# ChenWu98/cycle-diffusion

Measured on AMD Instinct MI355X. Metric: images/sec, SD-v1.4 512px CycleDiffusion 100+100 steps, 1/2/4/8 MI355X, higher is better.
Workload: dtype fp16

## Files before the change

cycle-diffusion_amd/csrc/capi_ops.hip:

```cpp
#include "capi_internal.h"

namespace {

bf16_t* op_rows16(cd_engine* h, const float* src, int64_t rows, int C) {
  bf16_t* d = (bf16_t*)h->arena.alloc((size_t)rows * C * 2);
  launch_nchw_to_nhwc(h->st, src, d, (int)rows, C, 1, C, 1.f, 0.f, 0);
  return d;
}
Act op_image16(Ctx& c, const float* x, int B, int C, int H, int W, int Cpad) {
  Act a = alloc_act(c, B, H, W, Cpad);
  launch_nchw_to_nhwc(c.st, x, a.p, B, C, H * W, Cpad, 1.f, 0.f, 0);
  return a;
}

bf16_t* op_nan_rows16(cd_engine* h, int64_t rows, int ld) {
  const size_t bytes = (size_t)(rows + 64) * ld * 2;
  bf16_t* t = (bf16_t*)h->arena.alloc(bytes);
  HIP_CHECK(hipMemsetAsync(t, 0xFF, bytes, h->st));
  return t;
}
float* op_nan_buffer(cd_engine* h, size_t n) {
  float* t = (float*)h->arena.alloc(n * sizeof(float));
  launch_fill_f32(h->st, t, __builtin_nanf(""), (int64_t)n);
  return t;
// ... 11 lines not shown

Act op_rows_view(const void* p, int B, int T, int C, int ld, bool f32) {
  Act a; a.p = (bf16_t*)const_cast<void*>(p); a.B = B; a.H = T; a.W = 1; a.C = C; a.ld = ld; a.f32 = f32;
  return a;
}
Act op_upload_rows(cd_engine* h, const float* x, int64_t rows, int C, int pad) {
  const int ld = C + pad;
  float* t = op_nan_buffer(h, (size_t)rows * ld);
  op_put_cols(h, t, ld, 0, x, rows, C);
  return op_rows_view(t, (int)rows, 1, C, ld, true);
}

const float* op_nchw_guarded(cd_engine* h, const float* x, int B, int C, int Czero, int ld, int HW) {
  if (ld == C) return x;
  float* t = op_nan_buffer(h, (size_t)B * ld * HW);
  if (Czero > C)
    HIP_CHECK(hipMemset2DAsync(t + (size_t)C * HW, (size_t)ld * HW * 4, 0, (size_t)(Czero - C) * HW * 4, B, h->st));
  HIP_CHECK(hipMemcpy2DAsync(t, (size_t)ld * HW * 4, x, (size_t)C * HW * 4, (size_t)C * HW * 4, B, hipMemcpyDeviceToDevice,
                             h->st));
  return t;
}
Act op_upload_nhwc(cd_engine* h, const float* x, int B, int C, int Czero, int ld, int H, int W) {
  const int HW = H * W;
  Act a; a.B = B; a.H = H; a.W = W; a.C = Czero; a.ld = ld; a.f32 = true;
  a.p = (bf16_t*)h->arena.alloc((size_t)B * HW * ld * sizeof(float));
  launch_nchw_to_nhwc_f32(h->st, op_nchw_guarded(h, x, B, C, Czero, ld, HW), a.pf(), B, ld, HW, ld, 1.f, 0.f);
  return a;
}
Act op_upload_nhwc16(cd_engine* h, const float* x, int B, int C, int ld, int H, int W, int Czero = 0) {
  const int HW = H * W;
  if (Czero < C) Czero = C;
  Act a; a.B = B; a.H = H; a.W = W; a.C = C; a.ld = ld;
  a.p = (bf16_t*)h->arena.alloc((size_t)B * HW * ld * sizeof(bf16_t));
  launch_nchw_to_nhwc(h->st, op_nchw_guarded(h, x, B, C, Czero, ld, HW), a.p, B, ld, HW, ld, 1.f, 0.f, 0);
  return a;
}
Act op_upload_nhwc_split(cd_engine* h, const float* x, int B, int C, int Cpad, int H, int W) {
  Act a; a.B = B; a.H = H; a.W = W; a.C = Cpad; a.ld = 2 * Cpad; a.f32 = true; a.split = true;
  a.p = (bf16_t*)h->arena.alloc((size_t)B * H * W * 2 * Cpad * sizeof(bf16_t));
  launch_nchw_to_nhwc_f32(h->st, x, a.pf(), B, C, H * W, Cpad, 1.f, 0.f, 1, h->overflow_dev);
  return a;
}

void op_download_nchw(cd_engine* h, const void* p, bool f32, int ld, float* y, int B, int C, int HW) {
  launch_nhwc_to_nchw(h->st, p, f32 ? 1 : 0, ld, y, B, C, HW, 1.f, 0.f);
}
void op_download(cd_engine* h, const Act& o, size_t floats, void* y) {
  HIP_CHECK(hipMemcpyAsync(y, o.p, floats * 4, hipMemcpyDeviceToDevice, h->st));
  HIP_CHECK(hipStreamSynchronize(h->st));
  h->check_overflow();
}

void conv_out_hw(int H, int W, int KH, int KW, int stride, int pad, bool asym, bool up, int* Ho, int* Wo) {
  const int Hin = up ? 2 * H : H, Win = up ? 2 * W : W;
  *Ho = asym ? (Hin + 1 - KH) / stride + 1 : (Hin + 2 * pad - KH) / stride + 1;
  *Wo = asym ? (Win + 1 - KW) / stride + 1 : (Win + 2 * pad - KW) / stride + 1;
}
Ctx prec_ctx(cd_engine* h, int precision) {
  Ctx c = h->ctx();
  c.f32 = precision != 0; c.x3 = precision == 2;
  return c;
}

void op_conv2d(cd_handle h, const float* x0, int C0, const float* x1, int C1, int B, int H, int W,
               const void* packed_w, int N, int KH, int KW, int stride, int pad, int asym_pad, int up,
               const float* bias, const float* rowvec, const float* resid, int act, int tile, bool out16,
               float* y, float* stats) {
  CD_CHECK(h && x0 && packed_w && y, "bad argument");
  ArenaScope arena_scope(h->arena);
  Ctx c = h->ctx();
  if (up && out16) {
    ConvW* pw = (ConvW*)const_cast<void*>(packed_w);
    h->op_params.add_up_phase(pw);
    h->op_params.refresh_up_phase(h->st, pw);
  }
  ConvW w = *(const ConvW*)packed_w;
  CD_CHECK(w.N == N && w.KH == KH && w.KW == KW, "packed weight does not match the call");
  w.b = const_cast<float*>(bias);
  Act a0 = op_image16(c, x0, B, C0, H, W, x1 ? C0 : round_up(C0, 32));
  Act a1;
  if (x1) a1 = op_image16(c, x1, B, C1, H, W, C1);
  ConvOpts o; o.stride = stride; o.pad = pad; o.asym = asym_pad != 0; o.up = up != 0; o.tile = tile;
  if (act & 0x400) {
    CD_CHECK(out16 && conv_ln_fold_available(c, w, (int64_t)B * H * W) , "LayerNorm fold needs tile 30 shapes");
    o.ln_fold = true;
    act &= ~0x400;
  }
  o.act = act;
  o.out_f32 = !out16;
  o.want_stats = stats != nullptr;
  int Ho, Wo;
  conv_out_hw(H, W, KH, KW, stride, pad, asym_pad != 0, up != 0, &Ho, &Wo);
  const int Nout = w.geglu ? N / 2 : N;
  if (rowvec) { o.rowvec = rowvec; o.rowvec_ld = N; o.rows_per_vec = Ho * Wo; }
  Act r;
  if (resid) {
    r = op_image16(c, resid, B, Nout, Ho, Wo, Nout);
    o.resid = &r;
  }
  Act out = conv_fwd(c, w, a0, x1 ? &a1 : nullptr, o);
  op_download_nchw(h, out.p, !out16, out.ld, y, B, Nout, Ho * Wo);
  if (stats) {
    CD_CHECK(out.stats, "this convolution produces no GroupNorm statistics (GEGLU, or rows %% 32 != 0)");
    HIP_CHECK(hipMemcpyAsync(stats, out.stats, (size_t)(out.rows() / 32) * 2 * Nout * sizeof(float),
                             hipMemcpyDeviceToDevice, h->st));
  }
}

void op_cross_attention_ctrl(cd_engine* h, const float* q_own, const float* q_src, const float* k_own,
                             const float* k_src, const float* v_own, const float* mapper, const float* alpha,
                             const float* weight, int B, int B_src, int B_ctrl, int H, int Tq, int L, int L_buf, int D,
                             float scale, int q_log2, int opad, float* o) {
  CD_CHECK(h && q_own && q_src && k_own && k_src && v_own && mapper && alpha && weight && o, "bad argument");
  CD_CHECK(B > 0 && B_src > 0 && B_ctrl > 0 && H > 0 && Tq > 0 && D > 0 && L > 0 && L_buf >= L, "bad argument");
  CD_CHECK(opad >= 0 && opad % 4 == 0, "opad: a multiple of 4 elements");
  ArenaScope arena_scope(h->arena);
  const int C = H * D, ldo = C + opad;
  CtrlAttnParams p;
  p.q_own = op_rows16(h, q_own, (int64_t)B * Tq, C); p.q_src = op_rows16(h, q_src, (int64_t)B_src * Tq, C);
  p.k_own = op_rows16(h, k_own, (int64_t)B * L_buf, C); p.k_src = op_rows16(h, k_src, (int64_t)B_src * L_buf, C);
  const bf16_t* vb16 = op_rows16(h, v_own, (int64_t)B * L, C);
  bf16_t* va = (bf16_t*)h->arena.alloc((size_t)B * L * C * 2);
  bf16_t* vb = (bf16_t*)h->arena.alloc((size_t)B * L * C * 2);
  launch_ctrl_values(h->st, vb16, mapper, alpha, weight, B, B_ctrl, L, C, va, vb);
  bf16_t* ob = op_nan_rows16(h, (int64_t)B * Tq, ldo);
  p.va = va; p.vb = vb; p.o = ob;
  p.B = B; p.B_src = B_src; p.H = H; p.Tq = Tq; p.L = L; p.D = D;
  p.ldq = C; p.ldk = C; p.ldv = C; p.ldo = ldo;
  p.q_bs = (int64_t)Tq * C; p.k_bs = (int64_t)L_buf * C; p.v_bs = (int64_t)L * C; p.o_bs = (int64_t)Tq * ldo;
  p.scale = scale; p.q_log2 = q_log2 != 0;
  launch_cross_attention_ctrl(h->st, p);
  op_download_nchw(h, ob, false, ldo, o, B * Tq, ldo, 1);
}

}

extern "C" {

int cd_op_pack_conv_weight(cd_handle h, const float* w_host, int N, int Cin, int KH, int KW, int geglu,
                           void** packed_dev, int* Npad, int* Cpad) {
  CD_API_BEGIN
  enter_engine(h);
  CD_CHECK(h && w_host && packed_dev, "bad argument");
  static int counter = 0;
  ConvW* c = h->op_params.new_conv(N, Cin, KH, KW, false, geglu != 0);
  const std::string name = "op." + std::to_string(counter++);
  h->op_params.conv_weight(name, c);
  int64_t shape[4] = {N, Cin, KH, KW};
  h->op_params.load(h->st, name, w_host, 4, shape);
  *packed_dev = c;
  if (Npad) *Npad = c->Npad;
  if (Cpad) *Cpad = c->Cpad;
  CD_API_END
}

int cd_op_free(cd_handle, void*) { return 0; }

int cd_op_conv2d(cd_handle h, const float* x0, int C0, const float* x1, int C1, int B, int H, int W,
                 const void* packed_w, int N, int KH, int KW, int stride, int pad, int asym_pad, int up,
                 const float* bias, const float* rowvec, const float* resid, int act, int tile, float* y) {
  CD_API_BEGIN
  enter_engine(h);
  op_conv2d(h, x0, C0, x1, C1, B, H, W, packed_w, N, KH, KW, stride, pad, asym_pad, up, bias, rowvec, resid, act, tile,
            false, y, nullptr);
  CD_API_END
}

// ... 973 lines not shown
```

cycle-diffusion_amd/csrc/engine.h:

```cpp
#pragma once
#include <map>
#include <memory>
#include <string>
#include <vector>

#include "common.h"
#include "kernels.h"
#include "../../include/cyclediff.h"

namespace cd {

class Arena {
 public:
  ~Arena();
  void init(size_t bytes);
  void* alloc(size_t bytes);
  size_t mark() const { return off_; }
  void release(size_t m) { off_ = m; }
  void reset() { off_ = 0; }
  size_t capacity() const { return cap_; }
  size_t high_water() const { return high_; }
 private:
  char* base_ = nullptr;
  size_t cap_ = 0, off_ = 0, high_ = 0;
// ... 48 lines not shown
  ~ParamStore();
  bool f32 = false;
  bool x3 = false;
  int* overflow = nullptr;
  int version = 0;
  ConvW* new_conv(int N, int Cin, int KH, int KW, bool bias, bool geglu = false);
  float* new_vec(int n, float init = 0.f);
  void add_up_phase(ConvW* c);
  void refresh_up_phase(hipStream_t st, ConvW* c);
  ParamDecl& declare(const std::string& name, std::vector<int64_t> shape);
  void conv_weight(const std::string& name, ConvW* c, int ref_ndim = 0, float scale = 1.f);
  void conv_weight_t(const std::string& name, ConvW* c);
  void conv_bias(const std::string& name, ConvW* c);
  void conv_rows(const std::string& name, std::vector<int64_t> shape, ConvW* c, int dst_row0, int rows,
                 int src_base, int grp, int grp_stride, float scale = 1.f);
  void bias_rows(const std::string& name, int64_t n_total, float* dst, int dst_off, int rows, int src_base,
                 int grp, int grp_stride);
  void vec(const std::string& name, float* dst, int n);
  void mat_f32(const std::string& name, float* dst, int N, int K, int dst_row0 = 0);

  void load(hipStream_t st, const std::string& name, const float* host, int ndim, const int64_t* shape);
  int missing(std::string* first = nullptr) const;
  const std::vector<std::unique_ptr<ParamDecl>>& decls() const { return decls_; }
  size_t device_bytes() const { return dev_bytes_; }
 private:
  std::vector<std::unique_ptr<ParamDecl>> decls_;
  std::map<std::string, ParamDecl*> by_name_;
  std::vector<std::unique_ptr<ConvW>> convs_;
  std::vector<void*> allocs_;
  float* staging_ = nullptr;
  size_t staging_bytes_ = 0;
  size_t dev_bytes_ = 0;
  void* dmalloc(size_t bytes);
};

struct Ctx {
  hipStream_t st = nullptr;
  Arena* arena = nullptr;
  const bf16_t* zeros = nullptr;
  float* gn_partial = nullptr;
  size_t gn_partial_floats = 0;
  bool f32 = false;
  bool x3 = false;
  int* overflow = nullptr;
};
class PrecisionScope {
 public:
  PrecisionScope(Ctx& c, bool f32, bool x3) : c_(c), f32_(c.f32), x3_(c.x3) { c.f32 = f32; c.x3 = x3; }
  ~PrecisionScope() { c_.f32 = f32_; c_.x3 = x3_; }
  PrecisionScope(const PrecisionScope&) = delete;
  PrecisionScope& operator=(const PrecisionScope&) = delete;
 private:
  Ctx& c_;
  const bool f32_, x3_;
};

struct ConvOpts {
  int stride = 1;
  int pad = 1;
  bool asym = false;
  bool up = false;
  const float* rowvec = nullptr; int rowvec_ld = 0; int rows_per_vec = 1;
  const Act* resid = nullptr;
  int act = ACT_NONE;
  float alpha = 1.f;
  bool out_f32 = false;
  void* out = nullptr;
  int out_ld = 0;
  bool ln_fold = false;
  float ln_eps = 1e-5f;
  bool raw_geglu = false;
  bool want_stats = false;
  float* out_stats = nullptr;
  int tile = 0;
};
Act attention_flash_f32_fwd(Ctx& c, const float* q, int ldq, const float* k, int ldk, int64_t k_bs, const float* v, int ldv,
                            int64_t v_bs, int B, int H, int Tq, int Tk, int D, float scale, int Himg, int Wimg, bool q_log2);
Act geglu_f32_fwd(Ctx& c, const Act& h);
Act split_rows_f32_fwd(Ctx& c, const Act& x, const Act* x2 = nullptr);
Act alloc_act(Ctx& c, int B, int H, int W, int C, bool with_stats = false);
Act conv_fwd(Ctx& c, const ConvW& w, const Act& x, const Act* x2, const ConvOpts& o);
bool conv_up_phase_taken(const Ctx& c, const ConvW& w, const Act& x, const Act* x2, const ConvOpts& o);
bool conv_ln_fold_available(const Ctx& c, const ConvW& w, int64_t rows);

struct GNW { float* g = nullptr; float* b = nullptr; int C = 0; float eps = 1e-5f; };
Act groupnorm_fwd(Ctx& c, const GNW& w, const Act& x, const Act* x2, bool silu, const float* film = nullptr,
                  int film_ld = 0);
struct LNW { float* g = nullptr; float* b = nullptr; int C = 0; };
Act layernorm_fwd(Ctx& c, const LNW& w, const Act& x);
const float* groupnorm_coef_fwd(Ctx& c, const GNW& w, const Act& x);
GNW make_gn(ParamStore& ps, const std::string& pfx, int C, float eps);
LNW make_ln(ParamStore& ps, const std::string& pfx, int C);
ConvW* make_conv(ParamStore& ps, const std::string& pfx, int N, int Cin, int k, bool bias = true, bool geglu = false,
                 int ref_ndim = 4, float wscale = 1.f);
Act net_input_act(const void* p, int B, int H, int W, int C, bool f32, bool x3);

struct ResW {
  int cin = 0, cout = 0;
  bool up = false, down = false, film = false;
  GNW gn1, gn2;
  ConvW *conv1 = nullptr, *conv2 = nullptr, *skip = nullptr;
  int emb_off = -1;
};
Act res_fwd(Ctx& c, const ResW& r, const Act& x, const Act* x2, const float* proj, int proj_ld, bool t_shared);

struct AttnW {
  int C = 0, heads = 1;
  GNW norm;
  ConvW *qk = nullptr, *v = nullptr, *proj = nullptr;
  float* vbias = nullptr;
};
Act attn_block_fwd(Ctx& c, const AttnW& a, const Act& x);

enum {
  ST_ENTRY_QKV = 1,
  ST_ENTRY_LN1 = 2,
  ST_ENTRY_GN = 4,
};
int st_entry_stages();
bool st_entry_available(const Ctx& c, int64_t rows, int hw);
constexpr int64_t kStEntryNetMinRows = 61440;
struct StEntryW {
  GNW norm; LNW ln1;
  const ConvW *proj_in = nullptr, *qk1 = nullptr, *v1 = nullptr;
  ConvW *qkv = nullptr, *qkv_ln = nullptr;
  const float* vbias = nullptr;
};
void st_entry_alloc(ParamStore& ps, StEntryW& w);
void st_entry_refresh(hipStream_t st, StEntryW& w);
struct StEntryOut { Act h, qk; bf16_t* vt = nullptr; int Tpad = 0; int stages = 0; };
void vt_gemm_fwd(Ctx& c, const ConvW& wv, const bf16_t* x, int ldx, int B, int T, int Tpad, bf16_t* vt);
struct AtCoreOut { Act o; bf16_t* vt = nullptr; int Tpad = 0; int branch = 0; };
AtCoreOut at_core(Ctx& c, const ConvW& wv, const float* vbias, const Act& qk, const Act& n, int C, int heads, Act o = Act());
Act st_entry_proj_in(Ctx& c, const StEntryW& w, const Act& x, int stages);
StEntryOut st_entry_qkv(Ctx& c, const StEntryW& w, const Act& h, int stages);
StEntryOut st_entry_fwd(Ctx& c, const StEntryW& w, const Act& x, int stages);

Act avgpool2_fwd(Ctx& c, const Act& x);
Act upsample2_fwd(Ctx& c, const Act& x);
Act attention_f32_fwd(Ctx& c, const Act& qk, const Act& v, int H, int D, float scale, const float* obias);

Act attention_fwd(Ctx& c, const bf16_t* q, int ldq, const bf16_t* k, int ldk, const bf16_t* v, int ldv, int B,
                  int H, int Tq, int Tk, int D, float scale, int Himg, int Wimg, bool q_log2 = false, int rows = -1);
Act attention_vt_fwd(Ctx& c, const bf16_t* q, int ldq, const bf16_t* k, int ldk, const bf16_t* vt, int B,
                     int H, int Tq, int Tk, int Tpad, int D, float scale, int Himg, int Wimg, bool q_log2 = false,
                     const float* obias = nullptr, Act o = Act());

class Net {
 public:
  virtual ~Net() {}
  ParamStore params;
  cd_net_desc desc;
  bool f32 = false;
  bool x3 = false;
  void set_precision(const cd_net_desc& d) {
    f32 = d.precision == CD_PREC_F32 || d.precision == CD_PREC_F32X3;
    x3 = d.precision == CD_PREC_F32X3;
    params.f32 = f32; params.x3 = x3;
  }
  virtual int kind() const = 0;
};

struct TimeEmb {
  int mode = 0, dim = 0, hidden = 0;
  float *w0 = nullptr, *b0 = nullptr, *w1 = nullptr, *b1 = nullptr;
  float* proj_w = nullptr; float* proj_b = nullptr;
// ... 91 lines not shown
```

cycle-diffusion_amd/csrc/engine.hip:

```cpp
#include <limits.h>
#include <stdlib.h>

#include "engine.h"

#include <string.h>

namespace cd {

Arena::~Arena() { if (base_) (void)hipFree(base_); }
void Arena::init(size_t bytes) {
  if (base_) { (void)hipFree(base_); base_ = nullptr; }
  HIP_CHECK(hipMalloc((void**)&base_, bytes));
  cap_ = bytes; off_ = 0; high_ = 0;
}
void* Arena::alloc(size_t bytes) {
  size_t a = (off_ + 255) & ~(size_t)255;
  CD_CHECK(a + bytes <= cap_, "workspace arena exhausted: need %zu more bytes (capacity %zu); "
           "create the engine with a larger workspace", a + bytes - cap_, cap_);
  off_ = a + bytes;
  if (off_ > high_) high_ = off_;
  return base_ + a;
}

ParamStore::~ParamStore() {
// ... 272 lines not shown
  p.wgt = w.wphase; p.Ktot = 4 * w.Cpad; p.N = w.N;
  p.alpha = o.alpha; p.bias = w.b;
  p.rowvec = o.rowvec; p.rowvec_ld = o.rowvec_ld; p.rows_per_vec = o.rows_per_vec;
  Act y; y.B = x.B; y.H = 2 * x.H; y.W = 2 * x.W; y.C = w.N; y.f32 = false;
  if (o.out) { y.p = (bf16_t*)o.out; y.ld = o.out_ld; }
  else { y.ld = w.N; y.p = (bf16_t*)c.arena->alloc((size_t)p.M * w.N * 2); }
  if (o.out && o.out_stats) y.stats_buf = o.out_stats;
  else if (!o.out && o.want_stats) y.stats_buf = (float*)c.arena->alloc((size_t)(p.M / 32) * 2 * w.N * sizeof(float));
  p.stats = y.stats_buf;
  y.stats = y.stats_buf;
  const size_t mk = c.arena->mark();
  bf16_t* tmp = (bf16_t*)c.arena->alloc((size_t)p.M * w.N * 2);
  p.out = tmp; p.out_ld = w.N;
  p.zeros = c.zeros; p.tile = o.tile;
  launch_conv_gemm(c.st, p);
  launch_up_phase_reorder(c.st, tmp, y.p, x.B, x.H, x.W, w.N, y.ld);
  c.arena->release(mk);
  return y;
}

Act conv_fwd(Ctx& c, const ConvW& w, const Act& x, const Act* x2, const ConvOpts& o) {
  if (conv_up_phase_taken(c, w, x, x2, o)) return conv_up_phase_fwd(c, w, x, o);
  if (x.split) {
    CD_CHECK(!x2, "conv: a split activation cannot be concatenated");
    return conv_split_fwd(c, w, x, o);
  }
  ConvGemmParams p;
  CD_CHECK(w.f32 == c.f32 && x.f32 == c.f32 && (!x2 || x2->f32 == c.f32) && (!o.resid || o.resid->f32 == c.f32),
           "conv: operand precision does not match the running network");
  CD_CHECK((!x2 || !x2->split) && (!o.resid || !o.resid->split), "conv: split activation as a second source / residual");
  p.src0 = x.p; p.C0 = round_up(x.C, 32); p.ld0 = x.ld;
  if (x2) {
    CD_CHECK(x2->B == x.B && x2->H == x.H && x2->W == x.W, "conv: concat sources differ in shape");
    p.src1 = x2->p; p.C1 = x2->C; p.ld1 = x2->ld;
    CD_CHECK(x.C % 32 == 0 && x2->C % 32 == 0, "conv: concat channels must be multiples of 32");
  }
  CD_CHECK(p.C0 + p.C1 == w.Cpad, "conv: input channels %d+%d do not match weight Cpad %d", p.C0, p.C1, w.Cpad);
  CD_CHECK(x.ld >= p.C0, "conv: source row shorter than padded channel count");
  p.B = x.B; p.Hs = x.H; p.Ws = x.W; p.up = o.up ? 1 : 0;
  p.Hin = o.up ? x.H * 2 : x.H; p.Win = o.up ? x.W * 2 : x.W;
  p.KH = w.KH; p.KW = w.KW; p.stride = o.stride;
  if (o.asym) { p.pad_t = 0; p.pad_l = 0; p.Hout = (p.Hin + 1 - w.KH) / o.stride + 1; p.Wout = (p.Win + 1 - w.KW) / o.stride + 1; }
  else {
    p.pad_t = o.pad; p.pad_l = o.pad;
    p.Hout = (p.Hin + 2 * o.pad - w.KH) / o.stride + 1;
    p.Wout = (p.Win + 2 * o.pad - w.KW) / o.stride + 1;
  }
  p.M = x.B * p.Hout * p.Wout;
  p.wgt = w.w; p.wgt_frag = w.wfrag; p.Ktot = w.Ktot(); p.N = w.N;
  p.alpha = o.alpha; p.bias = w.b;
  p.rowvec = o.rowvec; p.rowvec_ld = o.rowvec_ld; p.rows_per_vec = o.rows_per_vec;
  const bool fuse_geglu = w.geglu && !o.raw_geglu;
  p.act = fuse_geglu ? ACT_GEGLU : o.act;
  const int Nout = fuse_geglu ? w.N / 2 : w.N;
  Act y; y.B = x.B; y.H = p.Hout; y.W = p.Wout; y.C = Nout; y.f32 = c.f32;
  if (o.out) { y.p = (bf16_t*)o.out; y.ld = o.out_ld; }
  else {
    y.ld = Nout;
    y.p = (bf16_t*)c.arena->alloc((size_t)p.M * Nout * ((o.out_f32 || c.f32) ? 4 : 2));
  }
  if (o.resid) {
    CD_CHECK(o.resid->rows() == p.M && o.resid->C == Nout, "conv: residual shape mismatch");
    p.resid = o.resid->p; p.resid_ld = o.resid->ld;
  }
  p.out = y.p; p.out_ld = y.ld; p.out_f32 = o.out_f32 ? 1 : 0;
  p.zeros = c.zeros; p.tile = o.tile;
  if (o.ln_fold) { p.ln_fold = 1; p.ln_eps = o.ln_eps; p.tile = kLinStreamTile; }
  if (c.f32) {
    p.out_f32 = 1;
    launch_conv_gemm_f32(c.st, p);
    return y;
  }
  if (!w.geglu && !o.out_f32 && ((p.Hout * p.Wout) % 32) == 0) {
    if (o.out && o.out_stats) y.stats_buf = o.out_stats;
    else if (!o.out && o.want_stats)
      y.stats_buf = (float*)c.arena->alloc((size_t)(p.M / 32) * 2 * Nout * sizeof(float));
    p.stats = y.stats_buf;
    y.stats = y.stats_buf;
  }
  launch_conv_gemm(c.st, p);
  return y;
}

bool conv_ln_fold_available(const Ctx& c, const ConvW& w, int64_t rows) {
  static const bool on = [] { const char* e = getenv("CYCLEDIFF_LN_FOLD"); return !(e && e[0] == '0'); }();
  static const int64_t min_rows = [] { const char* e = getenv("CYCLEDIFF_LN_FOLD_MIN_ROWS"); return e ? atoll(e) : 32768ll; }();
  return on && !c.f32 && w.wfrag && w.KH == 1 && w.KW == 1 && w.Cpad == 320 && rows >= min_rows && rows % 32 == 0 &&
         w.N % 64 == 0 && w.N <= 2560;
}

Act groupnorm_fwd(Ctx& c, const GNW& w, const Act& x, const Act* x2, bool silu, const float* film,
                  int film_ld) {
  GroupNormParams p;
  p.x = x.p; p.C0 = x.C; p.ld0 = x.ld;
  if (x2) { p.x1 = x2->p; p.C1 = x2->C; p.ld1 = x2->ld; }
  const int C = p.C0 + p.C1;
  CD_CHECK(C == w.C, "groupnorm: channels %d != weight %d", C, w.C);
  p.B = x.B; p.HW = x.H * x.W; p.G = 32; p.eps = w.eps; p.gamma = w.g; p.beta = w.b;
  p.film = film; p.film_ld = film_ld; p.silu = silu ? 1 : 0;
  Act y = alloc_act(c, x.B, x.H, x.W, C);
  p.y = y.p;
  if (c.f32) {
    CD_CHECK(x.f32 && (!x2 || x2->f32) && !x.split && (!x2 || !x2->split), "groupnorm: operand precision");
    if (c.x3) { p.split_out = 1; p.overflow = c.overflow; y.split = true; y.ld = 2 * C; }
    if (x.stats && x.ld == x.C && (!x2 || (x2->stats && x2->ld == x2->C))) {
      p.pre0 = x.stats;
      p.pre1 = x2 ? x2->stats : nullptr;
    }
    const size_t mk = c.arena->mark();
    void* ws = c.arena->alloc(groupnorm_f32_workspace(p.B, p.HW, C));
    launch_groupnorm_f32(c.st, p, ws);
    c.arena->release(mk);
    return y;
  }
  p.S = groupnorm_slabs(p.B, p.HW, C);
  const size_t part_floats = round_up((size_t)p.B * p.S * p.G * 2, (size_t)64);
  CD_CHECK(part_floats + (size_t)p.B * 2 * C <= c.gn_partial_floats, "groupnorm: workspace too small");
  p.partial = c.gn_partial;
  p.coef = c.gn_partial + part_floats;
  if (x.stats && x.ld == x.C && (!x2 || (x2->stats && x2->ld == x2->C))) {
    p.pre0 = x.stats;
    p.pre1 = x2 ? x2->stats : nullptr;
  }
  launch_groupnorm(c.st, p);
  return y;
}

const float* groupnorm_coef_fwd(Ctx& c, const GNW& w, const Act& x) {
  CD_CHECK(!c.f32 && !x.f32 && !x.split && x.C == w.C, "groupnorm coefficients: 16-bit single source of %d channels", w.C);
  GroupNormParams p;
  p.x = x.p; p.C0 = x.C; p.ld0 = x.ld;
  p.B = x.B; p.HW = x.H * x.W; p.G = 32; p.eps = w.eps; p.gamma = w.g; p.beta = w.b;
  p.no_apply = 1;
  p.S = groupnorm_slabs(p.B, p.HW, x.C);
  const size_t part_floats = round_up((size_t)p.B * p.S * p.G * 2, (size_t)64);
  CD_CHECK(part_floats + (size_t)p.B * 2 * x.C <= c.gn_partial_floats, "groupnorm: workspace too small");
  p.partial = c.gn_partial;
  p.coef = c.gn_partial + part_floats;
  if (x.stats && x.ld == x.C) p.pre0 = x.stats;
  launch_groupnorm(c.st, p);
  return p.coef;
}

int st_entry_stages() {
  static const int v = [] {
    const char* e = getenv("CYCLEDIFF_ST_ENTRY");
    int s = e && e[0] ? atoi(e) : (ST_ENTRY_QKV | ST_ENTRY_LN1 | ST_ENTRY_GN);
    if (!(s & ST_ENTRY_QKV)) s &= ~ST_ENTRY_LN1;
    return s;
  }();
  return v;
}

bool st_entry_available(const Ctx& c, int64_t rows, int hw) {
  return !c.f32 && rows >= 32768 && lin_stream_entry_supports(rows, hw, 320);
}

void st_entry_alloc(ParamStore& ps, StEntryW& w) {
  if (!w.qk1 || !w.v1 || !w.qk1->wfrag || !w.v1->wfrag || w.qk1->Cpad != 320 || w.qk1->N != 640 || w.v1->N != 320) return;
  w.qkv = ps.new_conv(960, 320, 1, 1, true);
  w.qkv_ln = ps.new_conv(960, 320, 1, 1, true);
}

void st_entry_refresh(hipStream_t st, StEntryW& w) {
  if (!w.qkv) return;
  const size_t row = (size_t)320 * sizeof(bf16_t);
  HIP_CHECK(hipMemcpyAsync(w.qkv->w, w.qk1->w, 640 * row, hipMemcpyDeviceToDevice, st));
  HIP_CHECK(hipMemcpyAsync(w.qkv->w + (size_t)640 * 320, w.v1->w, 320 * row, hipMemcpyDeviceToDevice, st));
  HIP_CHECK(hipMemsetAsync(w.qkv->b, 0, 960 * sizeof(float), st));
  if (w.vbias) HIP_CHECK(hipMemcpyAsync(w.qkv->b + 640, w.vbias, 320 * sizeof(float), hipMemcpyDeviceToDevice, st));
  launch_pack_wfrag(st, w.qkv->w, 320, w.qkv->wfrag, 960);
// ... 329 lines not shown
```

cycle-diffusion_amd/csrc/lin_stream.hip:

```cpp
#include <stdlib.h>

#include <mutex>

#include "common.h"
#include "kernels.h"

namespace cd {
namespace lin_detail {

typedef __attribute__((address_space(3))) void* lptr_t;
typedef __attribute__((ext_vector_type(4))) unsigned int u32x4;

constexpr int K = 320, NKS = K / 16, KSH = NKS / 2;
constexpr int WPIECE = 2 * KSH * 1024, WSLOTS = 3;
constexpr int APIECE = 128 * 128, ASLOTS = 3;
constexpr int NAP = 10;
constexpr int ST_LD = 36, ST_BYTES = 32 * ST_LD * 4;
constexpr int BIAS_MAX = 2560;
constexpr int OFF_A = WSLOTS * WPIECE, OFF_ST = OFF_A + ASLOTS * APIECE, OFF_BIAS = OFF_ST + 8 * ST_BYTES;
constexpr int LDS_BYTES = OFF_BIAS + BIAS_MAX * 4;
static_assert(LDS_BYTES <= 160 * 1024, "LDS");
constexpr unsigned kNoLoad = 0x80000000u;

__device__ __forceinline__ void wait_vmcnt_le(int n) {
// ... 19 lines not shown
}

__device__ __forceinline__ u32x4 load16_hidden(u32x4 rsrc, unsigned voff) {
  u32x4 r;
  asm volatile("buffer_load_dwordx4 %0, %1, %2, 0 offen" : "=v"(r) : "v"(voff), "s"(rsrc) : "memory");
  return r;
}
__device__ __forceinline__ uint4 pack8_sat(const float* f) {
#if CD_ACT_FP16
  typedef __attribute__((ext_vector_type(2))) _Float16 h2;
  uint32_t w[4];
#pragma unroll
  for (int i = 0; i < 4; ++i) {
    const h2 v = {(_Float16)__builtin_amdgcn_fmed3f(f[2 * i], -65504.0f, 65504.0f),
                  (_Float16)__builtin_amdgcn_fmed3f(f[2 * i + 1], -65504.0f, 65504.0f)};
    w[i] = __builtin_bit_cast(uint32_t, v);
  }
  return make_uint4(w[0], w[1], w[2], w[3]);
#else
  return pack8(f);
#endif
}
__device__ __forceinline__ void touch4(u32x4& a, u32x4& b, u32x4& c, u32x4& d) {
  asm volatile("" : "+v"(a), "+v"(b), "+v"(c), "+v"(d)::"memory");
}

template <int ACT, bool RESID, bool STATS, bool LNF = false, bool VT = false, bool GNA = false>
__global__ __launch_bounds__(512, 2) void k_lin_stream(LinStreamParams p) {
#if defined(__HIP_DEVICE_COMPILE__)
  constexpr bool GEGLU = (ACT == ACT_GEGLU);
  static_assert(!(GEGLU && (RESID || STATS)), "GEGLU has neither residual nor statistics");
  static_assert(!(VT && (GEGLU || RESID || STATS)) && !(GNA && (LNF || VT)), "entry variants are plain projections");
  extern __shared__ __attribute__((aligned(16))) char smem[];
  char* wring = smem;
  char* aring = smem + OFF_A;
  const int tid = threadIdx.x, lane = tid & 63;
  const int wave = __builtin_amdgcn_readfirstlane(tid >> 6);
  float* stage = (float*)(smem + OFF_ST + wave * ST_BYTES);
  float* bias_s = (float*)(smem + OFF_BIAS);
  const int mi = lane & 31, half = lane >> 5;
  const bool w_issuer = wave < 4;
  const int wq = wave & 3;

  const int NT = p.N >> 6;
  const int I = 2 * NT;
  const int nstrips = (p.M + 255) >> 8;
  const int G = gridDim.x;
  const int my_count = (nstrips - (int)blockIdx.x + G - 1) / G;
  if (my_count <= 0) return;
  const int cs = I >= 80 ? 4 : (I >= 40 ? 2 : 1);

  const __amdgpu_buffer_rsrc_t rs_a =
      __builtin_amdgcn_make_buffer_rsrc((void*)p.a, 0, (unsigned)((size_t)p.M * p.lda * 2), 0x00020000);
  const __amdgpu_buffer_rsrc_t rs_w =
      __builtin_amdgcn_make_buffer_rsrc((void*)p.wfrag, 0, (unsigned)((size_t)p.N * K * 2), 0x00020000);
  const __amdgpu_buffer_rsrc_t rs_o = __builtin_amdgcn_make_buffer_rsrc(
      (void*)p.out, 0, (unsigned)((size_t)p.M * p.ldo * 2), 0x00020000);
  const __amdgpu_buffer_rsrc_t rs_v = __builtin_amdgcn_make_buffer_rsrc(
      (void*)(VT ? p.vt : p.out), 0, VT ? (unsigned)p.vt_bytes : 0u, 0x00020000);
  u32x4 rs_r = {0u, 0u, 0u, 0x00020000u};
  if (RESID) {
    const uint64_t ra = (uint64_t)p.resid;
    rs_r[0] = (unsigned)ra; rs_r[1] = (unsigned)(ra >> 32) & 0xffffu;
    rs_r[2] = (unsigned)((size_t)p.M * p.ldr * 2);
  }

  for (int i = tid; i < p.N; i += 512) bias_s[i] = p.bias ? p.bias[i] : 0.f;

  auto issue_a = [&](int row0, int j, int slot) {
    const unsigned a_row = (unsigned)((lane >> 3) * p.lda * 2);
#pragma unroll
    for (int u = 0; u < 4; ++u) {
      const int x = wq * 4 + u;
      const unsigned a_lane = a_row + (unsigned)(((lane & 7) ^ ((4 * u + (lane >> 4)) & 7)) * 16);
      const unsigned base = (unsigned)(((row0 + 128 * (j & 1) + 8 * x) * p.lda + (j >> 1) * 64) * 2);
      __builtin_amdgcn_raw_ptr_buffer_load_lds(rs_a, (lptr_t)(aring + slot * APIECE + x * 1024), 16, a_lane + base, 0,
                                               0, 0);
    }
  };
  int w_boff[5];
#pragma unroll
  for (int u = 0; u < 5; ++u) {
    const int x = wq + 4 * u;
    w_boff[u] = ((x / KSH) * NKS + (x % KSH)) * 1024;
  }
  auto issue_w = [&](int piece, bool valid, int slot) {
    const int base = ((piece >> 1) * 2 * NKS + (piece & 1) * KSH) * 1024;
    const unsigned voff = valid ? (unsigned)(lane * 16) : kNoLoad;
#pragma unroll
    for (int u = 0; u < 5; ++u)
      __builtin_amdgcn_raw_ptr_buffer_load_lds(rs_w, (lptr_t)(wring + slot * WPIECE + (wq + 4 * u) * 1024), 16, voff,
                                               base + w_boff[u], 0, 0);
  };

  bf16x8 af[NKS], afn[NKS];
  auto normalise_rows = [&]() __attribute__((always_inline)) {
    float s1 = 0.f, s2 = 0.f;
#pragma unroll
    for (int ks = 0; ks < NKS; ++ks) {
      float f[8];
      unpack8(__builtin_bit_cast(uint4, af[ks]), f);
#pragma unroll
      for (int e = 0; e < 8; ++e) { s1 += f[e]; s2 = __builtin_fmaf(f[e], f[e], s2); }
      __builtin_amdgcn_sched_barrier(0);
    }
    s1 += __shfl_xor(s1, 32);
    s2 += __shfl_xor(s2, 32);
    const float mean = s1 * (1.0f / K);
    const float var = fmaxf(s2 * (1.0f / K) - mean * mean, 0.f);
    const float rstd = __builtin_amdgcn_rsqf(var + p.ln_eps);
    const float nmr = -mean * rstd;
#pragma unroll
    for (int ks = 0; ks < NKS; ++ks) {
      float f[8];
      unpack8(__builtin_bit_cast(uint4, af[ks]), f);
#pragma unroll
      for (int e = 0; e < 8; ++e) f[e] = __builtin_fmaf(f[e], rstd, nmr);
      af[ks] = __builtin_bit_cast(bf16x8, pack8_sat(f));
      __builtin_amdgcn_sched_barrier(0);
    }
  };
  auto gn_apply_rows = [&](int row0) __attribute__((always_inline)) {
    typedef __attribute__((ext_vector_type(8))) float f32x8s;
    const float* cf = p.gn_coef + (int64_t)(row0 / p.hw) * (2 * K);
    const bool hi = (lane >> 5) != 0;
#pragma unroll
    for (int ks = 0; ks < NKS; ++ks) {
      float f[8], cc[2][8];
#pragma unroll
      for (int ab = 0; ab < 2; ++ab) {
        f32x8s c0, c1;
        if (ab == 0)
          asm volatile("s_load_dwordx8 %0, %2, %3\n\ts_load_dwordx8 %1, %2, %4\n\ts_waitcnt lgkmcnt(0)"
                       : "=&s"(c0), "=&s"(c1) : "s"(cf), "n"(ks * 64), "n"(ks * 64 + 32) : "memory");
        else
          asm volatile("s_load_dwordx8 %0, %2, %3\n\ts_load_dwordx8 %1, %2, %4\n\ts_waitcnt lgkmcnt(0)"
                       : "=&s"(c0), "=&s"(c1) : "s"(cf), "n"(K * 4 + ks * 64), "n"(K * 4 + ks * 64 + 32) : "memory");
#pragma unroll
        for (int e = 0; e < 8; ++e) {
          cc[ab][e] = hi ? c1[e] : c0[e];
          asm volatile("" : "+v"(cc[ab][e]));
        }
      }
      unpack8(__builtin_bit_cast(uint4, af[ks]), f);
#pragma unroll
      for (int e = 0; e < 8; ++e) f[e] = f[e] * cc[0][e] + cc[1][e];
      af[ks] = __builtin_bit_cast(bf16x8, pack8(f));
      asm volatile("" : "+v"(af[ks]));
      __builtin_amdgcn_sched_barrier(0);
    }
  };
  auto take_a = [&](int j, int slot) {
    if ((j & 1) != (wave >> 2)) return;
    const int row = wq * 32 + mi;
    const int sw = (row >> 1) & 7;
    unsigned base = (unsigned)(OFF_A + slot * APIECE + row * 128 + ((half ^ sw) << 4));
    asm volatile("" : "+v"(base));
    const int kb = j >> 1;
#pragma unroll
    for (int c = 0; c < 5; ++c) {
      if (kb == c) {
#pragma unroll
        for (int f = 0; f < 4; ++f) afn[4 * c + f] = *(const bf16x8*)(smem + (base ^ (unsigned)(32 * f)));
        asm volatile("" ::: "memory");
      }
    }
  };

  int seq = 0;
  int wm0 = 0, wm1 = 0;
// ... 8 lines not shown
    if (is_o < my_count && is_gi <= gi) {
      if (!w_issuer) {
        issue_a(is_row0, is_j, is_slot);
        seq += 4;
        am0 = a_fly == 0 ? seq : am0;
        am1 = a_fly == 0 ? am1 : seq;
      }
      const bool wrap = is_j == NAP - 1;
      const int step_in = is_o == 0 ? 1 : cs, step_wrap = is_o == 0 ? I - 12 * cs + 3 : I - 9 * cs;
      ++a_fly;
      ++e_issue;
      is_slot = is_slot == ASLOTS - 1 ? 0 : is_slot + 1;
      is_gi += wrap ? step_wrap : step_in;
      is_j = wrap ? 0 : is_j + 1;
      is_o += wrap ? 1 : 0;
      is_row0 += wrap ? G * 256 : 0;
    }
  };
  auto a_due = [&](int gi) { return e_cons < e_issue && cn_gi <= gi; };
  int ce_j = 0, ce_slot = 0;
  auto a_consume_step = [&]() {
    const bool wrap = cn_j == NAP - 1;
    const int step_in = cn_o == 0 ? 1 : cs, step_wrap = cn_o == 0 ? I - 10 * cs + 1 : I - 9 * cs;
    ce_j = cn_j; ce_slot = cn_slot;
    am0 = am1; --a_fly; ++e_cons;
    cn_slot = cn_slot == ASLOTS - 1 ? 0 : cn_slot + 1;
    cn_gi += wrap ? step_wrap : step_in;
    cn_j = wrap ? 0 : cn_j + 1;
    cn_o += wrap ? 1 : 0;
  };

  if (w_issuer) {
    issue_w(0, true, 0); seq += 5; wm0 = seq;
    issue_w(1, true, 1); seq += 5; wm1 = seq;
  }
  a_step_issue(-NAP - 2);
  a_step_issue(-NAP - 1);
  for (int gi = -NAP; gi < 0; ++gi) {
    const bool due = a_due(gi);
    if (due && !w_issuer) wait_vmcnt_le(seq - am0);
    asm volatile("s_waitcnt lgkmcnt(0)\n\ts_barrier" ::: "memory");
    if (due) a_consume_step();
    a_step_issue(gi);
    if (due) take_a(ce_j, ce_slot);
  }
#pragma unroll
  for (int ks = 0; ks < NKS; ++ks) af[ks] = afn[ks];
  if (GNA) gn_apply_rows((int)blockIdx.x * 256);
  if (LNF) normalise_rows();

  f32x16 acc[2];
  u32x4 rres[4];
  auto issue_resid = [&](int row0, int t) {
    if (!RESID || row0 + wave * 32 >= p.M) return;
    int l2 = lane;
    asm volatile("" : "+v"(l2));
    const unsigned r_lane = (unsigned)(((wave * 32 + (l2 >> 2)) * p.ldr + (l2 & 3) * 8) * 2);
#pragma unroll
    for (int nb = 0; nb < 2; ++nb)
#pragma unroll
      for (int ps = 0; ps < 2; ++ps) {
        const int soff = ((row0 + 16 * ps) * p.ldr + t * 64 + nb * 32) * 2;
        asm volatile("buffer_load_dwordx4 %0, %1, %2, %3 offen"
                     : "=v"(rres[nb * 2 + ps]) : "v"(r_lane), "s"(rs_r), "s"(soff) : "memory");
      }
    seq += 4;
    rmark = seq;
  };
  issue_resid((int)blockIdx.x * 256, 0);

  int gi = 0;
  int wslot = 0;
  for (int ord = 0; ord < my_count; ++ord) {
    const int row0 = ((int)blockIdx.x + ord * G) * 256;
    const bool has_next = ord + 1 < my_count;
    const bool rows_ok = row0 + wave * 32 < p.M;
    int vt_base = 0;
    if (VT) {
      const int img = row0 / p.hw;
      vt_base = img * (p.N - p.nsplit) * p.vt_ld + (row0 - img * p.hw) + wave * 32;
    }
    for (int t = 0; t < NT; ++t) {
#pragma unroll
      for (int r = 0; r < 16; ++r) { acc[0][r] = 0.f; acc[1][r] = 0.f; }
#pragma unroll
      for (int kh = 0; kh < 2; ++kh) {
        const int i = 2 * t + kh;
        if (w_issuer) wait_vmcnt_le(seq - wm0);
        const bool due = a_due(gi);
        if (due && !w_issuer) wait_vmcnt_le(seq - am0);
        asm volatile("s_waitcnt lgkmcnt(0)\n\ts_barrier" ::: "memory");
        if (w_issuer) {
          const int nxt = i + 2;
          const int slot2 = wslot == 0 ? 2 : wslot - 1;
          issue_w(nxt < I ? nxt : nxt - I, nxt < I || has_next, slot2);
          seq += 5;
          wm0 = wm1; wm1 = seq;
        }
        if (due) a_consume_step();
        a_step_issue(gi);
        const char* wp = wring + wslot * WPIECE + lane * 16;
        if (RESID) {
#pragma unroll
          for (int ksl = 0; ksl < KSH; ++ksl) {
            const bf16x8 w0 = *(const bf16x8*)(wp + ksl * 1024), w1 = *(const bf16x8*)(wp + (KSH + ksl) * 1024);
            acc[0] = CD_MFMA_32x32x16(w0, af[kh * KSH + ksl], acc[0]);
            acc[1] = CD_MFMA_32x32x16(w1, af[kh * KSH + ksl], acc[1]);
            __builtin_amdgcn_sched_barrier(0);
          }
        } else {
          constexpr int PFD = 2;
          bf16x8 wf[PFD + 1][2];
#pragma unroll
          for (int d = 0; d < PFD; ++d) {
            wf[d][0] = *(const bf16x8*)(wp + d * 1024);
            wf[d][1] = *(const bf16x8*)(wp + (KSH + d) * 1024);
          }
#pragma unroll
          for (int ksl = 0; ksl < KSH; ++ksl) {
            if (ksl + PFD < KSH) {
              wf[(ksl + PFD) % (PFD + 1)][0] = *(const bf16x8*)(wp + (ksl + PFD) * 1024);
              wf[(ksl + PFD) % (PFD + 1)][1] = *(const bf16x8*)(wp + (KSH + ksl + PFD) * 1024);
            }
            acc[0] = CD_MFMA_32x32x16(wf[ksl % (PFD + 1)][0], af[kh * KSH + ksl], acc[0]);
            acc[1] = CD_MFMA_32x32x16(wf[ksl % (PFD + 1)][1], af[kh * KSH + ksl], acc[1]);
            __builtin_amdgcn_sched_barrier(0);
          }
        }
        if (due) take_a(ce_j, ce_slot);
        wslot = wslot == 2 ? 0 : wslot + 1;
        ++gi;
      }
      if (RESID && rows_ok) {
        wait_vmcnt_le(seq - rmark);
        touch4(rres[0], rres[1], rres[2], rres[3]);
      }
      int l2 = lane;
      asm volatile("" : "+v"(l2));
      const int prow = l2 >> 2, pcol = (l2 & 3) * 8, mi2 = l2 & 31, half2 = l2 >> 5;
      const unsigned o_lane = (unsigned)(((wave * 32 + prow) * p.ldo + pcol) * 2);
      if constexpr (GEGLU) {
        const unsigned od_lane = (unsigned)(((wave * 32 + mi2) * p.ldo + 4 * half2) * 2);
#pragma unroll
        for (int q = 0; q < 4; ++q) {
          const float* bp = bias_s + t * 64 + 8 * q + 4 * half2;
          const f32x4 bv = *(const f32x4*)bp, bg = *(const f32x4*)(bp + 32);
          float val[4], gate[4], o4[4];
#pragma unroll
          for (int j = 0; j < 4; ++j) { val[j] = acc[0][4 * q + j] + bv[j]; gate[j] = acc[1][4 * q + j] + bg[j]; }
          mul_gelu4(val, gate, o4);
          if (rows_ok) {
            typedef __attribute__((ext_vector_type(2))) unsigned int u32x2;
            const u32x2 o = {pack2(o4[0], o4[1]), pack2(o4[2], o4[3])};
            __builtin_amdgcn_raw_buffer_store_b64(o, rs_o, od_lane, (row0 * p.ldo + t * 32 + 8 * q) * 2, 0);
          }
          __builtin_amdgcn_sched_barrier(0);
        }
      } else if (VT && t * 64 >= p.nsplit) {
        const unsigned v_lane = (unsigned)((prow * p.vt_ld + pcol) * 2);
#pragma unroll
        for (int nb = 0; nb < 2; ++nb) {
          __builtin_amdgcn_wave_barrier();
          const int ncol0 = t * 64 + nb * 32;
#pragma unroll
          for (int q = 0; q < 4; ++q) {
            const f32x4 bv = *(const f32x4*)(bias_s + ncol0 + 8 * q + 4 * half2);
#pragma unroll
            for (int j = 0; j < 4; ++j) stage[(8 * q + 4 * half2 + j) * ST_LD + mi2] = acc[nb][4 * q + j] + bv[j];
          }
          asm volatile("s_waitcnt lgkmcnt(0)" ::: "memory");
          __builtin_amdgcn_wave_barrier();
#pragma unroll
          for (int ps = 0; ps < 2; ++ps) {
            const float* srow = stage + (prow + 16 * ps) * ST_LD + pcol;
            const f32x4 lo = *(const f32x4*)srow, hi = *(const f32x4*)(srow + 4);
            const float v[8] = {lo[0], lo[1], lo[2], lo[3], hi[0], hi[1], hi[2], hi[3]};
            if (rows_ok) {
              const uint4 o = pack8_sat(v);
              __builtin_amdgcn_raw_buffer_store_b128(__builtin_bit_cast(u32x4, o), rs_v, v_lane,
                                                     (vt_base + (ncol0 - p.nsplit + 16 * ps) * p.vt_ld) * 2, 0);
            }
            __builtin_amdgcn_sched_barrier(0);
          }
        }
      } else {
#pragma unroll
      for (int nb = 0; nb < 2; ++nb) {
        __builtin_amdgcn_wave_barrier();
#pragma unroll
        for (int q = 0; q < 4; ++q) {
          const f32x4 v4 = {acc[nb][4 * q], acc[nb][4 * q + 1], acc[nb][4 * q + 2], acc[nb][4 * q + 3]};
          *(f32x4*)(stage + mi2 * ST_LD + 8 * q + 4 * half2) = v4;
        }
        asm volatile("s_waitcnt lgkmcnt(0)" ::: "memory");
        __builtin_amdgcn_wave_barrier();
        const int ncol0 = t * 64 + nb * 32;
        const f32x4 b0 = *(const f32x4*)(bias_s + ncol0 + pcol), b1 = *(const f32x4*)(bias_s + ncol0 + pcol + 4);
#pragma unroll
        for (int ps = 0; ps < 2; ++ps) {
          float* srow = stage + (prow + 16 * ps) * ST_LD + pcol;
          const f32x4 lo = *(const f32x4*)srow, hi = *(const f32x4*)(srow + 4);
          float v[8] = {lo[0] + b0[0], lo[1] + b0[1], lo[2] + b0[2], lo[3] + b0[3],
                        hi[0] + b1[0], hi[1] + b1[1], hi[2] + b1[2], hi[3] + b1[3]};
          if (RESID && rows_ok) {
            float rr[8];
            unpack8(__builtin_bit_cast(uint4, rres[nb * 2 + ps]), rr);
#pragma unroll
            for (int e = 0; e < 8; ++e) v[e] += rr[e];
          }
          if (rows_ok) {
            const uint4 o = pack8_sat(v);
            __builtin_amdgcn_raw_buffer_store_b128(__builtin_bit_cast(u32x4, o), rs_o, o_lane,
                                                   ((row0 + 16 * ps) * p.ldo + ncol0) * 2, 0);
          }
          if (STATS) {
            *(f32x4*)srow = (f32x4){v[0], v[1], v[2], v[3]};
            *(f32x4*)(srow + 4) = (f32x4){v[4], v[5], v[6], v[7]};
            asm volatile("s_waitcnt lgkmcnt(0)" ::: "memory");
          }
          __builtin_amdgcn_sched_barrier(0);
        }
        if (STATS) {
          __builtin_amdgcn_wave_barrier();
          float s1 = 0.f, s2 = 0.f;
#pragma unroll
          for (int r = 0; r < 16; ++r) {
            const float x = stage[(16 * half2 + r) * ST_LD + mi2];
            s1 += x; s2 += x * x;
          }
          s1 += __shfl_xor(s1, 32); s2 += __shfl_xor(s2, 32);
          if (rows_ok && half2 == 0) {
            float* sp = p.stats + (int64_t)((row0 + wave * 32) >> 5) * 2 * p.N + ncol0 + mi2;
            sp[0] = s1; sp[p.N] = s2;
// ... 176 lines not shown
```

Baseline: 3.682.

## Interleave GEGLU gate GELU with value-half MFMAs in LN-fold linear stream kernel

In the GEGLU path of the streaming linear kernel, the gate half of the weights is now computed first (swapped piece order and per-k-slice contiguous layout). Its bias-add and GELU are then applied element by element between the MFMAs of the value half, so the epilogue only does a multiply-add. This hides the transcendental gate work behind matrix-core issue and shortens the epilogue. A separate supported-check lets explicit LN-fold calls bypass the env and min-rows gating. The interleaving relies on a fixed mapping between MFMA steps and accumulator registers, which could misbehave if NKS differs from the assumed pattern.

```diff
diff --git a/cycle-diffusion_amd/csrc/capi_ops.hip b/cycle-diffusion_amd/csrc/capi_ops.hip
--- a/cycle-diffusion_amd/csrc/capi_ops.hip
+++ b/cycle-diffusion_amd/csrc/capi_ops.hip
@@ -117,7 +117,7 @@
   if (x1) a1 = op_image16(c, x1, B, C1, H, W, C1);
   ConvOpts o; o.stride = stride; o.pad = pad; o.asym = asym_pad != 0; o.up = up != 0; o.tile = tile;
   if (act & 0x400) {
-    CD_CHECK(out16 && conv_ln_fold_available(c, w, (int64_t)B * H * W) , "LayerNorm fold needs tile 30 shapes");
+    CD_CHECK(out16 && conv_ln_fold_supported(c, w, (int64_t)B * H * W), "LayerNorm fold needs tile 30 shapes");
     o.ln_fold = true;
     act &= ~0x400;
   }
diff --git a/cycle-diffusion_amd/csrc/engine.h b/cycle-diffusion_amd/csrc/engine.h
--- a/cycle-diffusion_amd/csrc/engine.h
+++ b/cycle-diffusion_amd/csrc/engine.h
@@ -154,6 +154,7 @@
 Act conv_fwd(Ctx& c, const ConvW& w, const Act& x, const Act* x2, const ConvOpts& o);
 bool conv_up_phase_taken(const Ctx& c, const ConvW& w, const Act& x, const Act* x2, const ConvOpts& o);
 bool conv_ln_fold_available(const Ctx& c, const ConvW& w, int64_t rows);
+bool conv_ln_fold_supported(const Ctx& c, const ConvW& w, int64_t rows);
 
 struct GNW { float* g = nullptr; float* b = nullptr; int C = 0; float eps = 1e-5f; };
 Act groupnorm_fwd(Ctx& c, const GNW& w, const Act& x, const Act* x2, bool silu, const float* film = nullptr,
diff --git a/cycle-diffusion_amd/csrc/engine.hip b/cycle-diffusion_amd/csrc/engine.hip
--- a/cycle-diffusion_amd/csrc/engine.hip
+++ b/cycle-diffusion_amd/csrc/engine.hip
@@ -378,11 +378,15 @@
   return y;
 }
 
+bool conv_ln_fold_supported(const Ctx& c, const ConvW& w, int64_t rows) {
+  return !c.f32 && w.wfrag && w.KH == 1 && w.KW == 1 && w.Cpad == 320 && rows % 32 == 0 && w.N % 64 == 0 &&
+         w.N <= 2560;
+}
+
 bool conv_ln_fold_available(const Ctx& c, const ConvW& w, int64_t rows) {
   static const bool on = [] { const char* e = getenv("CYCLEDIFF_LN_FOLD"); return !(e && e[0] == '0'); }();
   static const int64_t min_rows = [] { const char* e = getenv("CYCLEDIFF_LN_FOLD_MIN_ROWS"); return e ? atoll(e) : 32768ll; }();
-  return on && !c.f32 && w.wfrag && w.KH == 1 && w.KW == 1 && w.Cpad == 320 && rows >= min_rows && rows % 32 == 0 &&
-         w.N % 64 == 0 && w.N <= 2560;
+  return on && rows >= min_rows && conv_ln_fold_supported(c, w, rows);
 }
 
 Act groupnorm_fwd(Ctx& c, const GNW& w, const Act& x, const Act* x2, bool silu, const float* film,
diff --git a/cycle-diffusion_amd/csrc/lin_stream.hip b/cycle-diffusion_amd/csrc/lin_stream.hip
--- a/cycle-diffusion_amd/csrc/lin_stream.hip
+++ b/cycle-diffusion_amd/csrc/lin_stream.hip
@@ -125,10 +125,11 @@
 #pragma unroll
   for (int u = 0; u < 5; ++u) {
     const int x = wq + 4 * u;
-    w_boff[u] = ((x / KSH) * NKS + (x % KSH)) * 1024;
+    w_boff[u] = GEGLU ? x * 1024 : ((x / KSH) * NKS + (x % KSH)) * 1024;
   }
   auto issue_w = [&](int piece, bool valid, int slot) {
-    const int base = ((piece >> 1) * 2 * NKS + (piece & 1) * KSH) * 1024;
+    const int base = GEGLU ? ((piece >> 1) * 2 + ((piece & 1) ^ 1)) * NKS * 1024
+                           : ((piece >> 1) * 2 * NKS + (piece & 1) * KSH) * 1024;
     const unsigned voff = valid ? (unsigned)(lane * 16) : kNoLoad;
 #pragma unroll
     for (int u = 0; u < 5; ++u)
@@ -303,7 +304,10 @@
     }
     for (int t = 0; t < NT; ++t) {
 #pragma unroll
-      for (int r = 0; r < 16; ++r) { acc[0][r] = 0.f; acc[1][r] = 0.f; }
+      for (int r = 0; r < 16; ++r) {
+        if (!GEGLU) acc[0][r] = 0.f;
+        acc[1][r] = 0.f;
+      }
 #pragma unroll
       for (int kh = 0; kh < 2; ++kh) {
         const int i = 2 * t + kh;
@@ -321,7 +325,37 @@
         if (due) a_consume_step();
         a_step_issue(gi);
         const char* wp = wring + wslot * WPIECE + lane * 16;
-        if (RESID) {
+        if constexpr (GEGLU) {
+          constexpr int PFD = 2;
+          bf16x8 wf[PFD + 1];
+#pragma unroll
+          for (int d = 0; d < PFD; ++d) wf[d] = *(const bf16x8*)(wp + d * 1024);
+          const float* bgp = bias_s;
+          f32x4 bg[2];
+          if (kh == 1) {
+            int l3 = lane;
+            asm volatile("" : "+v"(l3));
+            bgp = bias_s + t * 64 + 32 + 4 * (l3 >> 5);
+            bg[0] = *(const f32x4*)bgp;
+#pragma unroll
+            for (int r = 0; r < 16; ++r) acc[0][r] = 0.f;
+          }
+#pragma unroll
+          for (int ks = 0; ks < NKS; ++ks) {
+            if (ks + PFD < NKS) wf[(ks + PFD) % (PFD + 1)] = *(const bf16x8*)(wp + (ks + PFD) * 1024);
+            acc[1 - kh] = CD_MFMA_32x32x16(wf[ks % (PFD + 1)], af[ks], acc[1 - kh]);
+            if (kh == 1 && ks % 5 != 4) {
+              const int r = ks - ks / 5;
+              if ((r & 3) == 0 && r < 12) bg[((r >> 2) + 1) & 1] = *(const f32x4*)(bgp + 8 * ((r >> 2) + 1));
+              float x = acc[1][r];
+              asm volatile("" : "+v"(x));
+              x = gelu_fast(x + bg[(r >> 2) & 1][r & 3]);
+              asm volatile("" : "+v"(x));
+              acc[1][r] = x;
+            }
+            __builtin_amdgcn_sched_barrier(0);
+          }
+        } else if (RESID) {
 #pragma unroll
           for (int ksl = 0; ksl < KSH; ++ksl) {
             const bf16x8 w0 = *(const bf16x8*)(wp + ksl * 1024), w1 = *(const bf16x8*)(wp + (KSH + ksl) * 1024);
@@ -364,12 +398,10 @@
         const unsigned od_lane = (unsigned)(((wave * 32 + mi2) * p.ldo + 4 * half2) * 2);
 #pragma unroll
         for (int q = 0; q < 4; ++q) {
-          const float* bp = bias_s + t * 64 + 8 * q + 4 * half2;
-          const f32x4 bv = *(const f32x4*)bp, bg = *(const f32x4*)(bp + 32);
-          float val[4], gate[4], o4[4];
-#pragma unroll
-          for (int j = 0; j < 4; ++j) { val[j] = acc[0][4 * q + j] + bv[j]; gate[j] = acc[1][4 * q + j] + bg[j]; }
-          mul_gelu4(val, gate, o4);
+          const f32x4 bv = *(const f32x4*)(bias_s + t * 64 + 8 * q + 4 * half2);
+          float o4[4];
+#pragma unroll
+          for (int j = 0; j < 4; ++j) o4[j] = (acc[0][4 * q + j] + bv[j]) * acc[1][4 * q + j];
           if (rows_ok) {
             typedef __attribute__((ext_vector_type(2))) unsigned int u32x2;
             const u32x2 o = {pack2(o4[0], o4[1]), pack2(o4[2], o4[3])};
```

After: 3.648. Within noise of the previous version (-0.9%).
